# MIT-REALM/gcbf-pytorch

Hardware: NVIDIA H100
Metric: agent*steps/sec (train step, device-timed) (higher is better)
Workload: dtype f32 via 3xfp16 tensor-core products (fp32 accumulate)

## Files before the change

### gcbf-pytorch_b200/csrc/gemm_wgmma_f16.cu

```cuda
#include <cuda.h>
#include <cuda_fp16.h>
#include <stdlib.h>

#include <atomic>

#include "common.cuh"
#include "sm90_ptx.cuh"

namespace gcbf {
namespace th {

using namespace ptx;

constexpr int BM = 128;
constexpr int BK = 32;
constexpr int SUB_N = 128;
constexpr int WG_K = 16;
constexpr int NUM_THREADS = 384;
constexpr int EPI_THREADS = 256;
constexpr int KCH_MAX = 256 / BK;
constexpr int MN_BOX = 64;
constexpr int A_BYTES = BM * BK * 2;
constexpr int B_BYTES = SUB_N * BK * 2;
constexpr int RING_BYTES = 128 * 1024;
template <int P> __host__ __device__ constexpr int stage_bytes() { return P == 3 ? 2 * A_BYTES + 2 * B_BYTES : A_BYTES + B_BYTES; }
template <int P> __host__ __device__ constexpr int stages() { return RING_BYTES / stage_bytes<P>(); }
constexpr int PARK_PITCH = SUB_N + 8;
constexpr int PARK_BYTES = BM * PARK_PITCH * 4;
static_assert(PARK_BYTES <= RING_BYTES, "the second half of a 256-wide tile is parked in the stage ring");
static_assert(2 * stages<1>() * 8 + (256 / 32) * 4 <= 256, "barriers and reduction words fit their 256 bytes");
constexpr int SMEM_BYTES = RING_BYTES + PARK_BYTES + 1024  + 256 ;

enum { EPI_FWD = 0, EPI_DGRAD = 1, EPI_WGRAD = 2 };

struct EpiParams {
  int mode;
  const float* alpha;
  const float* bias;
  int act;
  const float* relu_src;
  int ld_relu;
  const __half* relu_hi;
  int ld_relu_h;
  int accumulate;
  size_t split_stride;
  const uint32_t* amax_a; int a_sr, a_sc;
  const uint32_t* amax_b; int b_sr, b_sc;
  uint32_t* amax_out;
  __half* out_h;
  int ld_out_h;
  uint32_t* out_tile_amax;
  int out_amax_stride;
  float* colsum;
};

__host__ __device__ __forceinline__ uint32_t scale_bits_from_amax(uint32_t amax_bits) {
  const int e = (int)((amax_bits >> 23) & 0xffu);
  if (e == 0 || e == 255) return 0x3f800000u;
  int se = 127 + 14 - (e - 127);
  se = se < 2 ? 2 : (se > 252 ? 252 : se);
  return (uint32_t)se << 23;
}
__host__ __device__ __forceinline__ uint32_t inv_pow2_bits(uint32_t s_bits) { return (uint32_t)(254 - (int)(s_bits >> 23)) << 23; }

template <bool MN_MAJOR>
__device__ __forceinline__ uint64_t tile_desc(uint32_t tile_addr, int kk) {
  if (MN_MAJOR) {
    return make_smem_desc(tile_addr + (uint32_t)(kk * WG_K * 128), BK * 128, 1024, 128);
  }
  return make_smem_desc(tile_addr + (uint32_t)(kk * WG_K * 2), 16, 8 * BK * 2, BK * 2);
}

template <bool MN_MAJOR>
__device__ __forceinline__ void load_tile(uint8_t* dst, const CUtensorMap* map, uint64_t* bar, int mn0, int k0, int rows) {
  if (MN_MAJOR) {
    for (int j = 0; j < rows / MN_BOX; ++j) tma_load_2d(dst + j * (BK * 128), map, bar, mn0 + j * MN_BOX, k0);
  } else {
    tma_load_2d(dst, map, bar, k0, mn0);
  }
}

__device__ __forceinline__ void epi_sync() { asm volatile("bar.sync 1, %0;" ::"n"(EPI_THREADS) : "memory"); }

template <int BN, bool A_MN, bool B_MN, int P>
__global__ void __launch_bounds__(NUM_THREADS, 1)
gemm_h_kernel(const __grid_constant__ CUtensorMap map_a_hi, const __grid_constant__ CUtensorMap map_a_lo,
              const __grid_constant__ CUtensorMap map_b_hi, const __grid_constant__ CUtensorMap map_b_lo,
              float* __restrict__ C, int ldc, int Mo, int No, int tiles_n, int kblocks_per_split, int kblocks_total, int KCH, EpiParams ep) {
  static_assert(P == 3 || P == 1, "products per k-slice: 3 (3xFP16) or 1 (fp16)");
  constexpr int STAGES = stages<P>();
  constexpr int STAGE_BYTES = stage_bytes<P>();
  constexpr int B_OFF = (P == 3 ? 2 : 1) * A_BYTES;
  constexpr int NSUB = BN / SUB_N;
  constexpr int MODE = A_MN ? EPI_WGRAD : (B_MN ? EPI_DGRAD : EPI_FWD);
  extern __shared__ uint8_t smem_raw[];
  uint8_t* smem = reinterpret_cast<uint8_t*>((reinterpret_cast<uintptr_t>(smem_raw) + 1023) & ~uintptr_t(1023));
  float* park0 = reinterpret_cast<float*>(smem + RING_BYTES);
  float* park1 = reinterpret_cast<float*>(smem);
  uint64_t* bars = reinterpret_cast<uint64_t*>(smem + RING_BYTES + PARK_BYTES);
  uint64_t* full = bars;
  uint64_t* empty = bars + STAGES;
  uint32_t* red = reinterpret_cast<uint32_t*>(bars + 2 * STAGES);

  const int warp = threadIdx.x >> 5, lane = threadIdx.x & 31;
  const int kb0 = blockIdx.y * kblocks_per_split;
  const int kb1 = min(kblocks_total, kb0 + kblocks_per_split);
  const int nkb = kb1 - kb0;
  const int m0 = (blockIdx.x / tiles_n) * BM, n0t = (blockIdx.x % tiles_n) * BN;

  if (threadIdx.x == 0) {
    tma_prefetch_desc(&map_a_hi);
    if (P == 3) tma_prefetch_desc(&map_a_lo);
    tma_prefetch_desc(&map_b_hi);
    if (P == 3) tma_prefetch_desc(&map_b_lo);
    for (int s = 0; s < STAGES; ++s) { mbar_init(&full[s], 1); mbar_init(&empty[s], 2); }
    fence_barrier_init();
  }
  __syncthreads();

  if (warp < 4) {
    setmaxnreg_dec<40>();
    if (threadIdx.x == 0) {
      int stage = 0;
      uint32_t phase = 0;
      for (int sub = 0; sub < NSUB; ++sub) {
        for (int kb = kb0; kb < kb1; ++kb) {
          mbar_wait(&empty[stage], phase ^ 1);
          uint8_t* st = smem + stage * STAGE_BYTES;
          mbar_expect_tx(&full[stage], STAGE_BYTES);
          load_tile<A_MN>(st, &map_a_hi, &full[stage], m0, kb * BK, BM);
          if (P == 3) load_tile<A_MN>(st + A_BYTES, &map_a_lo, &full[stage], m0, kb * BK, BM);
          load_tile<B_MN>(st + B_OFF, &map_b_hi, &full[stage], n0t + sub * SUB_N, kb * BK, SUB_N);
          if (P == 3) load_tile<B_MN>(st + B_OFF + B_BYTES, &map_b_lo, &full[stage], n0t + sub * SUB_N, kb * BK, SUB_N);
          if (++stage == STAGES) { stage = 0; phase ^= 1; }
        }
      }
    }
  } else {
    setmaxnreg_inc<232>();
    if (nkb > 0) {
      const int tid = threadIdx.x - 128;
      const int wg = tid >> 7;
      const int wl = (tid >> 5) & 3;
      const bool leader = (tid & 127) == 0;
      const uint32_t a_off = (uint32_t)wg * 4096u;
      const int nch = (nkb + KCH - 1) / KCH;
      int nchunks = NSUB * nch;
      asm("" : "+r"(nchunks));
      int stage = 0;
      uint32_t phase = 0;
      int held = -1;
      float cs_prev = 0.f;
      float acc[64], d0[64], d1[64];
#pragma unroll
      for (int j = 0; j < 64; ++j) acc[j] = 0.f;

      auto park_acc = [&](float* park) {
        const int r0 = wg * 64 + wl * 16 + (lane >> 2);
#pragma unroll
        for (int j = 0; j < 64; j += 4) {
          const int c = 8 * (j >> 2) + 2 * (lane & 3);
          *reinterpret_cast<float2*>(park + r0 * PARK_PITCH + c) = make_float2(acc[j], acc[j + 1]);
          *reinterpret_cast<float2*>(park + (r0 + 8) * PARK_PITCH + c) = make_float2(acc[j + 2], acc[j + 3]);
        }
      };
      auto promote = [&](float (&p)[64], float cs) {
#pragma unroll
        for (int j = 0; j < 64; ++j) fence_operand(p[j]);
#pragma unroll
        for (int j = 0; j < 64; ++j) acc[j] = __fmaf_rn(p[j], cs, acc[j]);
      };
      auto run_chunk = [&](float (&d)[64], float (&p)[64], int g) {
        const int sub = (NSUB > 1 && g >= nch) ? 1 : 0;
        const int kc = (g - sub * nch) * KCH;
        const int n0 = n0t + sub * SUB_N;
        const int kstart = (kb0 + kc) * BK;
        const int ia = A_MN ? (kstart >> 7) * ep.a_sr + (m0 >> 8) * ep.a_sc : (m0 >> 7) * ep.a_sr + (kstart >> 8) * ep.a_sc;
        const int ib = B_MN ? (kstart >> 7) * ep.b_sr + (n0 >> 8) * ep.b_sc : 0;
        const float cs = __uint_as_float(inv_pow2_bits(scale_bits_from_amax(__ldg(ep.amax_a + ia)))) *
                         __uint_as_float(inv_pow2_bits(scale_bits_from_amax(__ldg(ep.amax_b + ib))));
        const int kend = min(nkb, kc + KCH);
        for (int kb = kc; kb < kend; ++kb) {
          mbar_wait(&full[stage], phase);
          const uint32_t st = smem_u32(smem + stage * STAGE_BYTES);
          const uint32_t a_hi = st + a_off, a_lo = st + A_BYTES + a_off, b_hi = st + B_OFF, b_lo = st + B_OFF + B_BYTES;
#pragma unroll
          for (int j = 0; j < 64; ++j) fence_operand(d[j]);
          wgmma_fence();
#pragma unroll
          for (int kk = 0; kk < BK / WG_K; ++kk) {
            if constexpr (P == 3) {
              const uint64_t dah = tile_desc<A_MN>(a_hi, kk), dal = tile_desc<A_MN>(a_lo, kk);
              const uint64_t dbh = tile_desc<B_MN>(b_hi, kk), dbl = tile_desc<B_MN>(b_lo, kk);
              wgmma_m64n128k16_f16<A_MN ? 1 : 0, B_MN ? 1 : 0>(d, dal, dbh, (kb > kc || kk > 0) ? 1u : 0u);
              wgmma_m64n128k16_f16<A_MN ? 1 : 0, B_MN ? 1 : 0>(d, dah, dbl, 1u);
              wgmma_m64n128k16_f16<A_MN ? 1 : 0, B_MN ? 1 : 0>(d, dah, dbh, 1u);
            } else {
              const uint64_t dah = tile_desc<A_MN>(a_hi, kk), dbh = tile_desc<B_MN>(b_hi, kk);
              wgmma_m64n128k16_f16<A_MN ? 1 : 0, B_MN ? 1 : 0>(d, dah, dbh, (kb > kc || kk > 0) ? 1u : 0u);
            }
          }
          wgmma_commit();
          wgmma_wait<1>();
          if (held >= 0 && leader) mbar_arrive(&empty[held]);
          held = stage;
          if (++stage == STAGES) { stage = 0; phase ^= 1; }
          if (kb == kc && g > 0) {
            promote(p, cs_prev);
            if (NSUB > 1 && g == nch) {
              park_acc(park0);
#pragma unroll
              for (int j = 0; j < 64; ++j) acc[j] = 0.f;
            }
          }
        }
        cs_prev = cs;
      };
      auto finish = [&](float (&d)[64]) {
        wgmma_wait<0>();
        if (leader) mbar_arrive(&empty[held]);
        promote(d, cs_prev);
        if (NSUB > 1) epi_sync();
        park_acc(NSUB > 1 ? park1 : park0);
      };
      for (int g = 0;; g += 2) {
        run_chunk(d0, d1, g);
        if (g + 1 == nchunks) { finish(d0); break; }
        run_chunk(d1, d0, g + 1);
        if (g + 2 == nchunks) { finish(d1); break; }
      }
      epi_sync();

      constexpr int CG4 = BN / 4;
      constexpr int ROWS_PER_ITER = EPI_THREADS / CG4;
      const int cg = tid % CG4;
      const int c = cg * 4;
      const int col = n0t + c;
      float* const pk = (c < SUB_N ? park0 : park1) + (c & (SUB_N - 1));
      const float alpha = ep.alpha ? __ldg(ep.alpha) : 1.f;
      float bias4[4] = {0.f, 0.f, 0.f, 0.f};
      if (MODE == EPI_FWD && ep.bias) {
        const float inv_alpha = 1.f / alpha;
#pragma unroll
        for (int u = 0; u < 4; ++u) bias4[u] = (col + u < No) ? __ldg(ep.bias + col + u) * inv_alpha : 0.f;
      }
      float tmax = 0.f;
      for (int r = tid / CG4; r < BM; r += ROWS_PER_ITER) {
        const int row = m0 + r;
        float4* p = reinterpret_cast<float4*>(pk + r * PARK_PITCH);
        float v[4];
        const float4 s = *p;
        v[0] = s.x; v[1] = s.y; v[2] = s.z; v[3] = s.w;
#pragma unroll
        for (int u = 0; u < 4; ++u) {
          float y = (v[u] + bias4[u]) * alpha;
          if (MODE == EPI_FWD) {
            if (ep.act == GCBF_ACT_RELU) y = fmaxf(y, 0.f);
            else if (ep.act == GCBF_ACT_TANH) y = tanhf(y);
          }
          const bool ok = row < Mo && col + u < No;
          if (MODE == EPI_DGRAD && ok) {
            if (ep.relu_src) y = (__ldg(ep.relu_src + (size_t)row * ep.ld_relu + col + u) > 0.f) ? y : 0.f;
            else if (ep.relu_hi) y = (__half2float(ep.relu_hi[(size_t)row * ep.ld_relu_h + col + u]) > 0.f) ? y : 0.f;
          }
          v[u] = ok ? y : 0.f;
          tmax = fmaxf(tmax, fabsf(v[u]));
        }
        *p = make_float4(v[0], v[1], v[2], v[3]);
      }
      float s_tile = 1.f;
      if (MODE != EPI_WGRAD && ep.out_h) {
        const uint32_t wmax = __reduce_max_sync(0xffffffffu, __float_as_uint(tmax));
        if (lane == 0) red[tid >> 5] = wmax;
        epi_sync();
        uint32_t m = 0;
#pragma unroll
        for (int w = 0; w < EPI_THREADS / 32; ++w) m = max(m, red[w]);
        s_tile = __uint_as_float(scale_bits_from_amax(m));
        if (tid == 0 && m0 < Mo && n0t < No) ep.out_tile_amax[(size_t)(m0 >> 7) * ep.out_amax_stride + (n0t >> 8)] = m;
      }
      float out_max = 0.f;
      const bool vec_c = C && (ldc & 3) == 0 && (reinterpret_cast<uintptr_t>(C) & 15) == 0;
      const size_t plane = (size_t)Mo * ep.ld_out_h;
      for (int r = tid / CG4; r < BM; r += ROWS_PER_ITER) {
        const int row = m0 + r;
        if (row >= Mo || col >= No) continue;
        const float4 s = *reinterpret_cast<const float4*>(pk + r * PARK_PITCH);
        const float v[4] = {s.x, s.y, s.z, s.w};
        const int nv = min(4, No - col);
        if (C) {
          float* dst = C + (size_t)blockIdx.y * ep.split_stride + (size_t)row * ldc + col;
          if (ep.accumulate) {
#pragma unroll
            for (int u = 0; u < 4; ++u)
              if (u < nv) { const float o = v[u] + dst[u]; dst[u] = o; out_max = fmaxf(out_max, fabsf(o)); }
          } else if (vec_c && nv == 4) {
            *reinterpret_cast<float4*>(dst) = s;
          } else {
#pragma unroll
            for (int u = 0; u < 4; ++u)
              if (u < nv) dst[u] = v[u];
          }
        }
        if (MODE != EPI_WGRAD && ep.out_h) {
          const float y0 = v[0] * s_tile, y1 = v[1] * s_tile, y2 = v[2] * s_tile, y3 = v[3] * s_tile;
          const __half2 h01 = __floats2half2_rn(y0, y1), h23 = __floats2half2_rn(y2, y3);
          const float2 f01 = __half22float2(h01), f23 = __half22float2(h23);
          const __half2 l01 = __floats2half2_rn(__fsub_rn(y0, f01.x), __fsub_rn(y1, f01.y));
          const __half2 l23 = __floats2half2_rn(__fsub_rn(y2, f23.x), __fsub_rn(y3, f23.y));
          __half* dh = ep.out_h + (size_t)row * ep.ld_out_h + col;
          if (nv == 4) {
            *reinterpret_cast<uint2*>(dh) = make_uint2(*reinterpret_cast<const uint32_t*>(&h01), *reinterpret_cast<const uint32_t*>(&h23));
            *reinterpret_cast<uint2*>(dh + plane) = make_uint2(*reinterpret_cast<const uint32_t*>(&l01), *reinterpret_cast<const uint32_t*>(&l23));
          } else {
            const __half hs[4] = {__low2half(h01), __high2half(h01), __low2half(h23), __high2half(h23)};
            const __half ls[4] = {__low2half(l01), __high2half(l01), __low2half(l23), __high2half(l23)};
            for (int u = 0; u < nv; ++u) { dh[u] = hs[u]; dh[plane + u] = ls[u]; }
          }
        }
      }
      if (ep.amax_out && !ep.accumulate) out_max = fmaxf(out_max, tmax);
      if (MODE == EPI_DGRAD && ep.colsum) epi_sync();
      if (MODE == EPI_DGRAD && ep.colsum && tid < BN) {
        const float* pc = (tid < SUB_N ? park0 : park1) + (tid & (SUB_N - 1));
        float csum = 0.f;
#pragma unroll 8
        for (int r = 0; r < BM; ++r) csum += pc[r * PARK_PITCH];
        if (n0t + tid < No) ep.colsum[(size_t)(blockIdx.x / tiles_n) * No + n0t + tid] = csum;
      }
      if (ep.amax_out) {
        const uint32_t m = __reduce_max_sync(0xffffffffu, __float_as_uint(out_max));
        if (lane == 0 && m) atomicMax(ep.amax_out, m);
      }
    }
  }
}
__global__ void amax_kernel(const float* __restrict__ src, int ld, int rows, int cols, uint32_t* __restrict__ slot, int vec4) {
  float m = 0.f;
  if (vec4) {
    const int w = cols >> 2;
    for (int r = blockIdx.x; r < rows; r += gridDim.x) {
      const float4* p = reinterpret_cast<const float4*>(src + (size_t)r * ld);
      for (int c = threadIdx.x; c < w; c += blockDim.x) {
        const float4 x = __ldg(p + c);
        m = fmaxf(fmaxf(m, fmaxf(fabsf(x.x), fabsf(x.y))), fmaxf(fabsf(x.z), fabsf(x.w)));
      }
    }
  } else {
    for (int r = blockIdx.x; r < rows; r += gridDim.x)
      for (int c = threadIdx.x; c < cols; c += blockDim.x) m = fmaxf(m, fabsf(__ldg(src + (size_t)r * ld + c)));
  }
  const uint32_t w = __reduce_max_sync(0xffffffffu, __float_as_uint(m));
  __shared__ uint32_t part[32];
  if ((threadIdx.x & 31) == 0) part[threadIdx.x >> 5] = w;
  __syncthreads();
  if (threadIdx.x < 32) {
    uint32_t v = threadIdx.x < (blockDim.x >> 5) ? part[threadIdx.x] : 0u;
    v = __reduce_max_sync(0xffffffffu, v);
    if (threadIdx.x == 0 && v) atomicMax(slot, v);
  }
}

constexpr int SPLIT_ROWS = 64;
__global__ void split_h_kernel(const float* __restrict__ src, int ld, int rows, int cols, const uint32_t* __restrict__ amax,
                               __half* __restrict__ dst, int ld_h, float* __restrict__ colsum) {
  const float s = __uint_as_float(scale_bits_from_amax(__ldg(amax)));
  const int c = (blockIdx.x * 32 + threadIdx.x) * 2;
  const int r0 = blockIdx.y * SPLIT_ROWS;
  const size_t plane = (size_t)rows * ld_h;
  float s0 = 0.f, s1 = 0.f;
  if (c < cols) {
    const bool pair = (c + 1 < cols);
    const int r1 = min(rows, r0 + SPLIT_ROWS);
    for (int r = r0 + threadIdx.y; r < r1; r += blockDim.y) {
      const float* p = src + (size_t)r * ld + c;
      const float x0 = __ldg(p), x1 = pair ? __ldg(p + 1) : 0.f;
      const float y0 = x0 * s, y1 = x1 * s;
      const __half2 hi = __floats2half2_rn(y0, y1);
      const float2 hf = __half22float2(hi);
      const __half2 lo = __floats2half2_rn(__fsub_rn(y0, hf.x), __fsub_rn(y1, hf.y));
      __half* d = dst + (size_t)r * ld_h + c;
      if (pair) {
        *reinterpret_cast<__half2*>(d) = hi;
        *reinterpret_cast<__half2*>(d + plane) = lo;
      } else {
        d[0] = __low2half(hi);
        d[plane] = __low2half(lo);
      }
      s0 += x0; s1 += x1;
    }
  }
  if (colsum) {
    __shared__ float red[8][64];
    red[threadIdx.y][2 * threadIdx.x] = s0;
    red[threadIdx.y][2 * threadIdx.x + 1] = s1;
    __syncthreads();
    if (threadIdx.y == 0) {
      float t0 = 0.f, t1 = 0.f;
#pragma unroll
      for (int y = 0; y < 8; ++y) { t0 += red[y][2 * threadIdx.x]; t1 += red[y][2 * threadIdx.x + 1]; }
      if (c < cols) colsum[(size_t)blockIdx.y * cols + c] = t0;
      if (c + 1 < cols) colsum[(size_t)blockIdx.y * cols + c + 1] = t1;
    }
  }
}

__device__ __forceinline__ void split4(const float4 x, float s, uint2& hi, uint2& lo) {
  const float y0 = x.x * s, y1 = x.y * s, y2 = x.z * s, y3 = x.w * s;
  const __half2 h01 = __floats2half2_rn(y0, y1), h23 = __floats2half2_rn(y2, y3);
  const float2 f01 = __half22float2(h01), f23 = __half22float2(h23);
  const __half2 l01 = __floats2half2_rn(__fsub_rn(y0, f01.x), __fsub_rn(y1, f01.y));
  const __half2 l23 = __floats2half2_rn(__fsub_rn(y2, f23.x), __fsub_rn(y3, f23.y));
  hi.x = *reinterpret_cast<const uint32_t*>(&h01); hi.y = *reinterpret_cast<const uint32_t*>(&h23);
  lo.x = *reinterpret_cast<const uint32_t*>(&l01); lo.y = *reinterpret_cast<const uint32_t*>(&l23);
}

__global__ void __launch_bounds__(256) split_h4_kernel(const float* __restrict__ src, int ld, int rows, int cols,
                                                       const uint32_t* __restrict__ amax, __half* __restrict__ dst, int ld_h,
                                                       float* __restrict__ colsum) {
  const float s = __uint_as_float(scale_bits_from_amax(__ldg(amax)));
  const int c = (blockIdx.x * 32 + threadIdx.x) * 4;
  const int r0 = blockIdx.y * SPLIT_ROWS;
  const size_t plane = (size_t)rows * ld_h;
  float cs[4] = {0.f, 0.f, 0.f, 0.f};
  if (c < cols) {
    const int r1 = min(rows, r0 + SPLIT_ROWS);
    for (int r = r0 + threadIdx.y; r < r1; r += 32) {
      float4 x[4];
#pragma unroll
      for (int u = 0; u < 4; ++u)
        x[u] = (r + 8 * u < r1) ? __ldg(reinterpret_cast<const float4*>(src + (size_t)(r + 8 * u) * ld + c)) : make_float4(0.f, 0.f, 0.f, 0.f);
#pragma unroll
      for (int u = 0; u < 4; ++u) {
        if (r + 8 * u < r1) {
          uint2 hi, lo;
          split4(x[u], s, hi, lo);
          __half* d = dst + (size_t)(r + 8 * u) * ld_h + c;
          *reinterpret_cast<uint2*>(d) = hi;
          *reinterpret_cast<uint2*>(d + plane) = lo;
          cs[0] += x[u].x; cs[1] += x[u].y; cs[2] += x[u].z; cs[3] += x[u].w;
        }
      }
    }
  }
  if (colsum) {
    __shared__ float red[8][128];
#pragma unroll
    for (int j = 0; j < 4; ++j) red[threadIdx.y][4 * threadIdx.x + j] = cs[j];
    __syncthreads();
    if (threadIdx.y < 4) {
      const int col = threadIdx.y * 32 + threadIdx.x;
      float t = 0.f;
#pragma unroll
      for (int y = 0; y < 8; ++y) t += red[y][col];
      const int gc = blockIdx.x * 128 + col;
      if (gc < cols) colsum[(size_t)blockIdx.y * cols + gc] = t;
    }
  }
}

constexpr int kSplitMaxBatch = 16;
struct SplitBatch {
  const float* src[kSplitMaxBatch];
  uint32_t* amax[kSplitMaxBatch];
  __half* dst[kSplitMaxBatch];
  int ld[kSplitMaxBatch], rows[kSplitMaxBatch], cols[kSplitMaxBatch], ld_h[kSplitMaxBatch];
};

__global__ void __launch_bounds__(256) amax_batched_kernel(const __grid_constant__ SplitBatch b) {
  const int t = blockIdx.z;
  const int ld = b.ld[t], rows = b.rows[t], cols = b.cols[t];
  const int warp = threadIdx.x >> 5, lane = threadIdx.x & 31;
  const float* __restrict__ src = b.src[t];
  const bool vec = ((cols & 3) == 0 && (ld & 3) == 0 && (reinterpret_cast<uintptr_t>(src) & 15) == 0);
  float m = 0.f;
  for (int r = blockIdx.x * 8 + warp; r < rows; r += gridDim.x * 8) {
    const float* row = src + (size_t)r * ld;
    if (vec) {
      const float4* p = reinterpret_cast<const float4*>(row);
      for (int c = lane; c < (cols >> 2); c += 32) {
        const float4 x = __ldg(p + c);
        m = fmaxf(fmaxf(m, fmaxf(fabsf(x.x), fabsf(x.y))), fmaxf(fabsf(x.z), fabsf(x.w)));
      }
    } else {
      for (int c = lane; c < cols; c += 32) m = fmaxf(m, fabsf(__ldg(row + c)));
    }
  }
  const uint32_t w = __reduce_max_sync(0xffffffffu, __float_as_uint(m));
  __shared__ uint32_t part[8];
  if (lane == 0) part[warp] = w;
  __syncthreads();
  if (threadIdx.x < 32) {
    uint32_t v = threadIdx.x < 8 ? part[threadIdx.x] : 0u;
    v = __reduce_max_sync(0xffffffffu, v);
    if (threadIdx.x == 0 && v) atomicMax(b.amax[t], v);
  }
}

__global__ void __launch_bounds__(256) split_batched_kernel(const __grid_constant__ SplitBatch b) {
  const int t = blockIdx.z;
  const int ld = b.ld[t], rows = b.rows[t], cols = b.cols[t], ld_h = b.ld_h[t];
  const int c = (blockIdx.x * 32 + threadIdx.x) * 2;
  const int r0 = blockIdx.y * SPLIT_ROWS;
  if (c >= cols || r0 >= rows) return;
  const float* __restrict__ src = b.src[t];
  __half* __restrict__ dst = b.dst[t];
  const float s = __uint_as_float(scale_bits_from_amax(*b.amax[t]));
  const size_t plane = (size_t)rows * ld_h;
  const bool pair = (c + 1 < cols);
  const int r1 = min(rows, r0 + SPLIT_ROWS);
  for (int r = r0 + threadIdx.y; r < r1; r += blockDim.y) {
    const float* p = src + (size_t)r * ld + c;
    const float y0 = __ldg(p) * s, y1 = pair ? __ldg(p + 1) * s : 0.f;
    const __half2 hi = __floats2half2_rn(y0, y1);
    const float2 hf = __half22float2(hi);
    const __half2 lo = __floats2half2_rn(__fsub_rn(y0, hf.x), __fsub_rn(y1, hf.y));
    __half* d = dst + (size_t)r * ld_h + c;
    if (pair) {
      *reinterpret_cast<__half2*>(d) = hi;
      *reinterpret_cast<__half2*>(d + plane) = lo;
    } else {
      d[0] = __low2half(hi);
      d[plane] = __low2half(lo);
    }
  }
}

typedef CUresult (*EncodeTiledFn)(CUtensorMap*, CUtensorMapDataType, cuuint32_t, void*, const cuuint64_t*, const cuuint64_t*,
                                  const cuuint32_t*, const cuuint32_t*, CUtensorMapInterleave, CUtensorMapSwizzle,
                                  CUtensorMapL2promotion, CUtensorMapFloatOOBfill);

static EncodeTiledFn get_encode_fn() {
  static EncodeTiledFn fn = nullptr;
  if (!fn) {
    void* p = nullptr;
    cudaDriverEntryPointQueryResult q;
    if (cudaGetDriverEntryPoint("cuTensorMapEncodeTiled", &p, cudaEnableDefault, &q) == cudaSuccess && p) fn = (EncodeTiledFn)p;
  }
  return fn;
}

static int make_map(CUtensorMap* map, const __half* base, int rows, int cols, int ld_h, bool mn_major, int tile_rows) {
  EncodeTiledFn fn = get_encode_fn();
  if (!fn) { set_error("cuTensorMapEncodeTiled entry point unavailable"); return GCBF_E_CUDA; }
  cuuint64_t dims[2] = {(cuuint64_t)cols, (cuuint64_t)rows};
  cuuint64_t strides[1] = {(cuuint64_t)ld_h * 2};
  cuuint32_t box[2] = {(cuuint32_t)(mn_major ? MN_BOX : BK), (cuuint32_t)(mn_major ? BK : tile_rows)};
  cuuint32_t estr[2] = {1, 1};
  CUresult r = fn(map, CU_TENSOR_MAP_DATA_TYPE_FLOAT16, 2, const_cast<__half*>(base), dims, strides, box, estr,
                  CU_TENSOR_MAP_INTERLEAVE_NONE, mn_major ? CU_TENSOR_MAP_SWIZZLE_128B : CU_TENSOR_MAP_SWIZZLE_64B,
                  CU_TENSOR_MAP_L2_PROMOTION_L2_256B, CU_TENSOR_MAP_FLOAT_OOB_FILL_NONE);
  if (r != CUDA_SUCCESS) {
    set_error("cuTensorMapEncodeTiled failed (%d) rows=%d cols=%d ld=%d mn=%d", (int)r, rows, cols, ld_h, (int)mn_major);
    return GCBF_E_CUDA;
  }
  return GCBF_OK;
}

static std::atomic<long long> g_tc_launches[2];

static bool g_env_read = false;
static int g_kch = 4;
static int g_kch_dgrad = 8;

struct Operand {
  const __half* hi; int rows; int cols; int ld_h; bool mn_major;
  const __half* lo() const { return hi + (size_t)rows * ld_h; }
};
struct OutH {
  __half* hi; int rows; int cols; int ld_h; uint32_t* tile_amax; int amax_stride;
};

template <int BN, bool A_MN, bool B_MN, int P>
static int launch(const Operand& A, const Operand& B, float* C, int ldc, int Mo, int No, int Kc, int splits, EpiParams ep,
                  const OutH* oh, cudaStream_t st) {
  if (!g_env_read) {
    const char* kc = getenv("GCBF_TC_KCH");
    if (kc && atoi(kc) >= 1 && atoi(kc) <= KCH_MAX) g_kch = atoi(kc);
    const char* kd = getenv("GCBF_TC_KCH_DGRAD");
    if (kd && atoi(kd) >= 1 && atoi(kd) <= KCH_MAX) g_kch_dgrad = atoi(kd);
    if (kc && !kd) g_kch_dgrad = g_kch > 4 ? g_kch : g_kch_dgrad;
    g_env_read = true;
  }
  if ((ep.a_sr || ep.a_sc || ep.b_sr || ep.b_sc) && g_kch > 4) { set_error("tile-scaled operands need promotion chunks of <= 128 K-elements (GCBF_TC_KCH <= 4)"); return GCBF_E_UNSUPPORTED; }
  if constexpr (BN != 256 || A_MN) {
    if (oh || ep.colsum) { set_error("companion emission / column sums need a 256-wide forward or data-grad launch"); return GCBF_E_UNSUPPORTED; }
  }
  CUtensorMap mah, mal, mbh, mbl;
  if (int rc = make_map(&mah, A.hi, A.rows, A.cols, A.ld_h, A_MN, BM)) return rc;
  if (int rc = make_map(&mbh, B.hi, B.rows, B.cols, B.ld_h, B_MN, SUB_N)) return rc;
  if (P == 3) {
    if (int rc = make_map(&mal, A.lo(), A.rows, A.cols, A.ld_h, A_MN, BM)) return rc;
    if (int rc = make_map(&mbl, B.lo(), B.rows, B.cols, B.ld_h, B_MN, SUB_N)) return rc;
  } else {
    mal = mah; mbl = mbh;
  }
  if (oh) {
    ep.out_h = oh->hi; ep.ld_out_h = oh->ld_h; ep.out_tile_amax = oh->tile_amax; ep.out_amax_stride = oh->amax_stride;
  }
  static bool attr_set = false;
  if (!attr_set) {
    GCBF_CUDA_OK(cudaFuncSetAttribute(gemm_h_kernel<BN, A_MN, B_MN, P>, cudaFuncAttributeMaxDynamicSharedMemorySize, SMEM_BYTES));
    attr_set = true;
  }
  const int tiles_m = ceil_div(Mo, BM), tiles_n = ceil_div(No, BN);
  const int kblocks = ceil_div(Kc, BK);
  const int kch = (!A_MN && B_MN && !(ep.b_sr || ep.b_sc)) ? g_kch_dgrad : g_kch;
  const int kps = ceil_div(ceil_div(kblocks, splits), kch) * kch;
  const int nsplit = ceil_div(kblocks, kps);
  float* part = nullptr;
  float* colsum_part = nullptr;
  float* const colsum = ep.colsum;
  const int accumulate = ep.accumulate;
  if (nsplit > 1) {
    GCBF_CUDA_OK(scratch_alloc((void**)&part, (size_t)nsplit * Mo * No * 4, st));
    ep.split_stride = (size_t)Mo * No;
    ep.accumulate = 0;
  }
  if (colsum) {
    GCBF_CUDA_OK(scratch_alloc((void**)&colsum_part, (size_t)tiles_m * No * 4, st));
    ep.colsum = colsum_part;
  }
  gemm_h_kernel<BN, A_MN, B_MN, P><<<dim3(tiles_m * tiles_n, nsplit), NUM_THREADS, SMEM_BYTES, st>>>(mah, mal, mbh, mbl, part ? part : C,
                                                                                                    part ? No : ldc, Mo, No, tiles_n, kps,
                                                                                                    kblocks, kch, ep);
  GCBF_LAUNCH_OK();
  g_tc_launches[P == 1 ? 1 : 0].fetch_add(1, std::memory_order_relaxed);
  if (part) {
    GCBF_CUDA_OK(add_partials(part, nsplit, Mo, No, C, ldc, accumulate, st));
    GCBF_CUDA_OK(scratch_free(part, st));
  }
  if (colsum_part) {
    GCBF_CUDA_OK(add_partials(colsum_part, tiles_m, 1, No, colsum, No, 1, st));
    GCBF_CUDA_OK(scratch_free(colsum_part, st));
  }
  return GCBF_OK;
}

template <int BN, bool A_MN, bool B_MN>
static int launch_p(int products, const Operand& A, const Operand& B, float* C, int ldc, int Mo, int No, int Kc, int splits,
                    const EpiParams& ep, const OutH* oh, cudaStream_t st) {
  return products == 1 ? launch<BN, A_MN, B_MN, 1>(A, B, C, ldc, Mo, No, Kc, splits, ep, oh, st)
                       : launch<BN, A_MN, B_MN, 3>(A, B, C, ldc, Mo, No, Kc, splits, ep, oh, st);
}

static int check_plane(const void* p, int ld_h, const char* what) {
  if (!p || (reinterpret_cast<uintptr_t>(p) & 15) || (ld_h & 7)) {
    set_error("%s: fp16 companion must be 16-byte aligned with a pitch that is a multiple of 8 halves (ptr=%p ld=%d)", what, p, ld_h);
    return GCBF_E_INVALID;
  }
  return GCBF_OK;
}

}
}

using namespace gcbf;

extern "C" int gcbf_amax_f32(const float* src, int ld, int rows, int cols, void* amax_slot, int accumulate, void* stream) {
  GCBF_REQUIRE(amax_slot && rows >= 0 && cols >= 0 && ld >= cols, "gcbf_amax_f32: bad arguments rows=%d cols=%d ld=%d", rows, cols, ld);
  cudaStream_t st = as_stream(stream);
  if (!accumulate) GCBF_CUDA_OK(cudaMemsetAsync(amax_slot, 0, 4, st));
  if (rows == 0 || cols == 0) return GCBF_OK;
  GCBF_REQUIRE(src, "gcbf_amax_f32: null src");
  const int vec4 = ((cols & 3) == 0 && (ld & 3) == 0 && (reinterpret_cast<uintptr_t>(src) & 15) == 0) ? 1 : 0;
  const int work = vec4 ? cols / 4 : cols;
  const int threads = work >= 256 ? 256 : (work >= 128 ? 128 : 64);
  const int blocks = (int)imin64(rows, (int64_t)kNumSMs * (2048 / threads));
  th::amax_kernel<<<blocks, threads, 0, st>>>(src, ld, rows, cols, reinterpret_cast<uint32_t*>(amax_slot), vec4);
  GCBF_LAUNCH_OK();
  return GCBF_OK;
}

extern "C" int gcbf_split_f16(const float* src, int ld, int rows, int cols, const void* amax_slot, void* dst, int ld_h,
                              float* colsum, int colsum_accumulate, void* stream) {
  GCBF_REQUIRE(amax_slot && dst && rows >= 0 && cols >= 0 && ld >= cols && ld_h >= cols, "gcbf_split_f16: bad arguments rows=%d cols=%d", rows, cols);
  if (int rc = th::check_plane(dst, ld_h, "gcbf_split_f16")) return rc;
  cudaStream_t st = as_stream(stream);
  if (colsum && !colsum_accumulate) GCBF_CUDA_OK(cudaMemsetAsync(colsum, 0, (size_t)cols * 4, st));
  if (rows == 0 || cols == 0) return GCBF_OK;
  GCBF_REQUIRE(src, "gcbf_split_f16: null src");
  dim3 block(32, 8);
  const int strips = ceil_div(rows, th::SPLIT_ROWS);
  float* part = nullptr;
  if (colsum) GCBF_CUDA_OK(scratch_alloc((void**)&part, (size_t)strips * cols * 4, st));
  if ((cols & 3) == 0 && (ld & 3) == 0 && (reinterpret_cast<uintptr_t>(src) & 15) == 0) {
    dim3 grid(ceil_div(cols, 128), strips);
    th::split_h4_kernel<<<grid, block, 0, st>>>(src, ld, rows, cols, reinterpret_cast<const uint32_t*>(amax_slot),
                                               reinterpret_cast<__half*>(dst), ld_h, part);
  } else {
    dim3 grid(ceil_div(cols, 64), strips);
    th::split_h_kernel<<<grid, block, 0, st>>>(src, ld, rows, cols, reinterpret_cast<const uint32_t*>(amax_slot),
                                              reinterpret_cast<__half*>(dst), ld_h, part);
  }
  GCBF_LAUNCH_OK();
  if (part) {
    GCBF_CUDA_OK(add_partials(part, strips, 1, cols, colsum, cols, 1, st));
    GCBF_CUDA_OK(scratch_free(part, st));
  }
  return GCBF_OK;
}

extern "C" int gcbf_amax_split_batched(const gcbf_split_desc* descs, int count, void* stream) {
  GCBF_REQUIRE(descs && count >= 0, "gcbf_amax_split_batched: bad arguments");
  cudaStream_t st = as_stream(stream);
  for (int base = 0; base < count; base += th::kSplitMaxBatch) {
    const int nb = min(th::kSplitMaxBatch, count - base);
    th::SplitBatch b{};
    int max_rows = 0, max_cols = 0;
    for (int i = 0; i < nb; ++i) {
      const gcbf_split_desc& d = descs[base + i];
      GCBF_REQUIRE(d.src && d.amax_slot && d.dst && d.rows > 0 && d.cols > 0 && d.ld >= d.cols && d.ld_h >= d.cols,
                   "gcbf_amax_split_batched: descriptor %d", base + i);
      if (int rc = th::check_plane(d.dst, d.ld_h, "gcbf_amax_split_batched")) return rc;
      b.src[i] = d.src; b.amax[i] = reinterpret_cast<uint32_t*>(d.amax_slot); b.dst[i] = reinterpret_cast<__half*>(d.dst);
      b.ld[i] = d.ld; b.rows[i] = d.rows; b.cols[i] = d.cols; b.ld_h[i] = d.ld_h;
      max_rows = max(max_rows, d.rows); max_cols = max(max_cols, d.cols);
      GCBF_CUDA_OK(cudaMemsetAsync(d.amax_slot, 0, 4, st));
    }
    th::amax_batched_kernel<<<dim3(min(ceil_div(max_rows, 8), 8 * kNumSMs), 1, nb), 256, 0, st>>>(b);
    GCBF_LAUNCH_OK();
    th::split_batched_kernel<<<dim3(ceil_div(max_cols, 64), ceil_div(max_rows, th::SPLIT_ROWS), nb), dim3(32, 8), 0, st>>>(b);
    GCBF_LAUNCH_OK();
  }
  return GCBF_OK;
}

extern "C" long long gcbf_tc_launch_count(int products, int reset) {
  if (products != 1 && products != 3) { set_error("gcbf_tc_launch_count: products %d (3 or 1)", products); return -1; }
  std::atomic<long long>& c = th::g_tc_launches[products == 1 ? 1 : 0];
  return reset ? c.exchange(0) : c.load();
}

extern "C" int gcbf_linear_h_supported(int M, int N, int K) {
  return (M >= 256 && N >= 96 && K >= 96 && (long long)M * N * K >= (1ll << 24)) ? 1 : 0;
}

static int check_h16(const gcbf_h16* h, const char* what, int rows, int cols) {
  if (!h || !h->buf || !h->amax || h->rows != rows || h->cols != cols || h->ld < cols) {
    set_error("%s: companion descriptor (expected [%d x %d])", what, rows, cols);
    return GCBF_E_INVALID;
  }
  return th::check_plane(h->buf, h->ld, what);
}

extern "C" int gcbf_linear_fwd_tp(const gcbf_h16* X, const gcbf_h16* W, const float* bias, const float* inv_sigma, int act, float* Y, int ldy,
                                  const gcbf_h16* Yh, void* out_amax, int M, int N, int K, void* stream, int products) {
  GCBF_REQUIRE(M > 0 && N > 0 && K > 0 && (Y || Yh) && (!Y || ldy >= N), "gcbf_linear_fwd_t: bad arguments M=%d N=%d K=%d", M, N, K);
  GCBF_REQUIRE(products == 3 || products == 1, "gcbf_linear_fwd_tp: products %d (3 or 1)", products);
  if (int rc = check_h16(X, "gcbf_linear_fwd_t X", M, K)) return rc;
  if (int rc = check_h16(W, "gcbf_linear_fwd_t W", N, K)) return rc;
  GCBF_REQUIRE(W->amax_row_stride == 0 && W->amax_col_stride == 0, "gcbf_linear_fwd_t: the weight companion must be per-tensor scaled");
  cudaStream_t st = as_stream(stream);
  th::EpiParams ep{};
  ep.mode = th::EPI_FWD; ep.alpha = inv_sigma; ep.bias = bias; ep.act = act;
  ep.amax_a = reinterpret_cast<const uint32_t*>(X->amax); ep.a_sr = X->amax_row_stride; ep.a_sc = X->amax_col_stride;
  ep.amax_b = reinterpret_cast<const uint32_t*>(W->amax);
  ep.amax_out = reinterpret_cast<uint32_t*>(out_amax);
  if (out_amax) GCBF_CUDA_OK(cudaMemsetAsync(out_amax, 0, 4, st));
  th::OutH oh{};
  if (Yh) {
    if (int rc = check_h16(Yh, "gcbf_linear_fwd_t Yh", M, N)) return rc;
    GCBF_REQUIRE(N > 128 && Yh->amax_row_stride == ceil_div(N, 256) && Yh->amax_col_stride == 1, "gcbf_linear_fwd_t: emitted companions are tile-scaled (N > 128, amax strides (ceil(N/256), 1))");
    oh = th::OutH{reinterpret_cast<__half*>(Yh->buf), M, N, Yh->ld, reinterpret_cast<uint32_t*>(Yh->amax), Yh->amax_row_stride};
  }
  th::Operand A{reinterpret_cast<const __half*>(X->buf), M, K, X->ld, false}, B{reinterpret_cast<const __half*>(W->buf), N, K, W->ld, false};
  return (N > 128) ? th::launch_p<256, false, false>(products, A, B, Y, ldy, M, N, K, 1, ep, Yh ? &oh : nullptr, st)
                   : th::launch_p<128, false, false>(products, A, B, Y, ldy, M, N, K, 1, ep, nullptr, st);
}

extern "C" int gcbf_linear_fwd_t(const gcbf_h16* X, const gcbf_h16* W, const float* bias, const float* inv_sigma, int act, float* Y, int ldy,
                                 const gcbf_h16* Yh, void* out_amax, int M, int N, int K, void* stream) {
  return gcbf_linear_fwd_tp(X, W, bias, inv_sigma, act, Y, ldy, Yh, out_amax, M, N, K, stream, 3);
}

extern "C" int gcbf_linear_bwd_data_tp(const gcbf_h16* dZ, const gcbf_h16* W, const float* inv_sigma, const float* relu_src, int ld_relu,
                                       const gcbf_h16* relu_h, float* dX, int lddx, int accumulate, const gcbf_h16* dXh, float* colsum,
                                       void* out_amax, int M, int N, int K, void* stream, int products) {
  GCBF_REQUIRE(M > 0 && N > 0 && K > 0 && (dX || dXh) && (!dX || lddx >= K), "gcbf_linear_bwd_data_t: bad arguments M=%d N=%d K=%d", M, N, K);
  GCBF_REQUIRE(products == 3 || products == 1, "gcbf_linear_bwd_data_tp: products %d (3 or 1)", products);
  GCBF_REQUIRE(!relu_src || ld_relu >= K, "gcbf_linear_bwd_data_t: ld_relu");
  GCBF_REQUIRE(!(relu_src && relu_h) && !(accumulate && (dXh || colsum)), "gcbf_linear_bwd_data_t: conflicting options");
  if (int rc = check_h16(dZ, "gcbf_linear_bwd_data_t dZ", M, N)) return rc;
  if (int rc = check_h16(W, "gcbf_linear_bwd_data_t W", N, K)) return rc;
  GCBF_REQUIRE(W->amax_row_stride == 0 && W->amax_col_stride == 0, "gcbf_linear_bwd_data_t: the weight companion must be per-tensor scaled");
  if (relu_h) { if (int rc = check_h16(relu_h, "gcbf_linear_bwd_data_t relu_h", M, K)) return rc; }
  cudaStream_t st = as_stream(stream);
  th::EpiParams ep{};
  ep.mode = th::EPI_DGRAD; ep.alpha = inv_sigma; ep.relu_src = relu_src; ep.ld_relu = ld_relu; ep.accumulate = accumulate;
  if (relu_h) { ep.relu_hi = reinterpret_cast<const __half*>(relu_h->buf); ep.ld_relu_h = relu_h->ld; }
  ep.amax_a = reinterpret_cast<const uint32_t*>(dZ->amax); ep.a_sr = dZ->amax_row_stride; ep.a_sc = dZ->amax_col_stride;
  ep.amax_b = reinterpret_cast<const uint32_t*>(W->amax);
  ep.amax_out = reinterpret_cast<uint32_t*>(out_amax);
  ep.colsum = colsum;
  if (out_amax) GCBF_CUDA_OK(cudaMemsetAsync(out_amax, 0, 4, st));
  th::OutH oh{};
  if (dXh) {
    if (int rc = check_h16(dXh, "gcbf_linear_bwd_data_t dXh", M, K)) return rc;
    GCBF_REQUIRE(K > 128 && dXh->amax_row_stride == ceil_div(K, 256) && dXh->amax_col_stride == 1, "gcbf_linear_bwd_data_t: emitted companions are tile-scaled (K > 128, amax strides (ceil(K/256), 1))");
    oh = th::OutH{reinterpret_cast<__half*>(dXh->buf), M, K, dXh->ld, reinterpret_cast<uint32_t*>(dXh->amax), dXh->amax_row_stride};
  }
  th::Operand A{reinterpret_cast<const __half*>(dZ->buf), M, N, dZ->ld, false}, B{reinterpret_cast<const __half*>(W->buf), N, K, W->ld, true};
  return (K > 128) ? th::launch_p<256, false, true>(products, A, B, dX, lddx, M, K, N, 1, ep, dXh ? &oh : nullptr, st)
                   : th::launch_p<128, false, true>(products, A, B, dX, lddx, M, K, N, 1, ep, nullptr, st);
}

extern "C" int gcbf_linear_bwd_data_t(const gcbf_h16* dZ, const gcbf_h16* W, const float* inv_sigma, const float* relu_src, int ld_relu,
                                      const gcbf_h16* relu_h, float* dX, int lddx, int accumulate, const gcbf_h16* dXh, float* colsum,
                                      void* out_amax, int M, int N, int K, void* stream) {
  return gcbf_linear_bwd_data_tp(dZ, W, inv_sigma, relu_src, ld_relu, relu_h, dX, lddx, accumulate, dXh, colsum, out_amax, M, N, K, stream, 3);
}

extern "C" int gcbf_linear_bwd_weight_tp(const gcbf_h16* dZ, const gcbf_h16* X, const float* inv_sigma, float* dW, int lddw, int accumulate,
                                         int M, int N, int K, void* stream, int products) {
  GCBF_REQUIRE(M > 0 && N > 0 && K > 0 && lddw >= K && dW, "gcbf_linear_bwd_weight_t: bad arguments M=%d N=%d K=%d", M, N, K);
  GCBF_REQUIRE(products == 3 || products == 1, "gcbf_linear_bwd_weight_tp: products %d (3 or 1)", products);
  if (int rc = check_h16(dZ, "gcbf_linear_bwd_weight_t dZ", M, N)) return rc;
  if (int rc = check_h16(X, "gcbf_linear_bwd_weight_t X", M, K)) return rc;
  cudaStream_t st = as_stream(stream);
  th::EpiParams ep{};
  ep.mode = th::EPI_WGRAD; ep.alpha = inv_sigma; ep.accumulate = accumulate;
  ep.amax_a = reinterpret_cast<const uint32_t*>(dZ->amax); ep.a_sr = dZ->amax_row_stride; ep.a_sc = dZ->amax_col_stride;
  ep.amax_b = reinterpret_cast<const uint32_t*>(X->amax); ep.b_sr = X->amax_row_stride; ep.b_sc = X->amax_col_stride;
  const int BN = (K > 128) ? 256 : 128;
  const int tiles = ceil_div(N, th::BM) * ceil_div(K, BN);
  int splits = 1;
  if (tiles < kNumSMs) splits = max(1, min(ceil_div(M, 256), kNumSMs / tiles));
  th::Operand A{reinterpret_cast<const __half*>(dZ->buf), M, N, dZ->ld, true}, B{reinterpret_cast<const __half*>(X->buf), M, K, X->ld, true};
  return (BN == 256) ? th::launch_p<256, true, true>(products, A, B, dW, lddw, N, K, M, splits, ep, nullptr, st)
                     : th::launch_p<128, true, true>(products, A, B, dW, lddw, N, K, M, splits, ep, nullptr, st);
}

extern "C" int gcbf_linear_bwd_weight_t(const gcbf_h16* dZ, const gcbf_h16* X, const float* inv_sigma, float* dW, int lddw, int accumulate,
                                        int M, int N, int K, void* stream) {
  return gcbf_linear_bwd_weight_tp(dZ, X, inv_sigma, dW, lddw, accumulate, M, N, K, stream, 3);
}

static gcbf_h16 per_tensor(const void* buf, int ld, const void* amax, int rows, int cols) {
  gcbf_h16 h;
  h.buf = const_cast<void*>(buf); h.amax = const_cast<void*>(amax); h.ld = ld; h.rows = rows; h.cols = cols; h.amax_row_stride = 0; h.amax_col_stride = 0;
  return h;
}

extern "C" int gcbf_linear_fwd_h(const void* Xh, int ldxh, const void* x_amax, const void* Wh, int ldwh, const void* w_amax,
                                 const float* bias, const float* inv_sigma, float* Y, int ldy, int M, int N, int K, int act,
                                 void* out_amax, void* stream) {
  GCBF_REQUIRE(Y && x_amax && w_amax, "gcbf_linear_fwd_h: null pointer");
  const gcbf_h16 X = per_tensor(Xh, ldxh, x_amax, M, K), W = per_tensor(Wh, ldwh, w_amax, N, K);
  return gcbf_linear_fwd_t(&X, &W, bias, inv_sigma, act, Y, ldy, nullptr, out_amax, M, N, K, stream);
}

extern "C" int gcbf_linear_bwd_data_h(const void* dZh, int lddzh, const void* dz_amax, const void* Wh, int ldwh,
                                      const void* w_amax, const float* inv_sigma, const float* relu_src, int ld_relu, float* dX,
                                      int lddx, int M, int N, int K, int accumulate, void* out_amax, void* stream) {
  GCBF_REQUIRE(dX && dz_amax && w_amax, "gcbf_linear_bwd_data_h: null pointer");
  const gcbf_h16 dZ = per_tensor(dZh, lddzh, dz_amax, M, N), W = per_tensor(Wh, ldwh, w_amax, N, K);
  return gcbf_linear_bwd_data_t(&dZ, &W, inv_sigma, relu_src, ld_relu, nullptr, dX, lddx, accumulate, nullptr, nullptr, out_amax, M, N, K, stream);
}

extern "C" int gcbf_linear_bwd_weight_h(const void* dZh, int lddzh, const void* dz_amax, const void* Xh, int ldxh,
                                        const void* x_amax, const float* inv_sigma, float* dW, int lddw, int M, int N, int K,
                                        int accumulate, void* stream) {
  GCBF_REQUIRE(dW && dz_amax && x_amax, "gcbf_linear_bwd_weight_h: null pointer");
  const gcbf_h16 dZ = per_tensor(dZh, lddzh, dz_amax, M, N), X = per_tensor(Xh, ldxh, x_amax, M, K);
  return gcbf_linear_bwd_weight_t(&dZ, &X, inv_sigma, dW, lddw, accumulate, M, N, K, stream);
}
```

### gcbf-pytorch_b200/csrc/sm90_ptx.cuh

```cuda
#pragma once
#include <cuda.h>
#include <stdint.h>

namespace gcbf {
namespace ptx {

__device__ __forceinline__ uint32_t smem_u32(const void* p) { return (uint32_t)__cvta_generic_to_shared(p); }

__device__ __forceinline__ void mbar_init(uint64_t* bar, uint32_t count) {
  asm volatile("mbarrier.init.shared::cta.b64 [%0], %1;" ::"r"(smem_u32(bar)), "r"(count));
}
__device__ __forceinline__ void mbar_expect_tx(uint64_t* bar, uint32_t bytes) {
  asm volatile("mbarrier.arrive.expect_tx.shared::cta.b64 _, [%0], %1;" ::"r"(smem_u32(bar)), "r"(bytes) : "memory");
}
__device__ __forceinline__ void mbar_arrive(uint64_t* bar) {
  asm volatile("mbarrier.arrive.shared::cta.b64 _, [%0];" ::"r"(smem_u32(bar)) : "memory");
}
__device__ __forceinline__ uint32_t mbar_try_wait(uint64_t* bar, uint32_t parity) {
  uint32_t ok;
  asm volatile(
      "{\n\t"
      ".reg .pred p;\n\t"
      "mbarrier.try_wait.parity.shared::cta.b64 p, [%1], %2;\n\t"
      "selp.u32 %0, 1, 0, p;\n\t"
      "}"
      : "=r"(ok)
      : "r"(smem_u32(bar)), "r"(parity)
      : "memory");
  return ok;
}
__device__ __forceinline__ void mbar_wait(uint64_t* bar, uint32_t parity) {
  while (!mbar_try_wait(bar, parity)) {
  }
}
__device__ __forceinline__ void fence_barrier_init() { asm volatile("fence.mbarrier_init.release.cluster;" ::: "memory"); }

__device__ __forceinline__ void tma_load_2d(void* smem_dst, const CUtensorMap* map, uint64_t* bar, int c0, int c1) {
  asm volatile(
      "cp.async.bulk.tensor.2d.shared::cluster.global.mbarrier::complete_tx::bytes [%0], [%1, {%3, %4}], [%2];" ::"r"(
          smem_u32(smem_dst)),
      "l"(reinterpret_cast<uint64_t>(map)), "r"(smem_u32(bar)), "r"(c0), "r"(c1)
      : "memory");
}
__device__ __forceinline__ void tma_prefetch_desc(const CUtensorMap* map) {
  asm volatile("prefetch.tensormap [%0];" ::"l"(reinterpret_cast<uint64_t>(map)) : "memory");
}

__device__ __forceinline__ void wgmma_fence() { asm volatile("wgmma.fence.sync.aligned;" ::: "memory"); }
__device__ __forceinline__ void wgmma_commit() { asm volatile("wgmma.commit_group.sync.aligned;" ::: "memory"); }
template <int N>
__device__ __forceinline__ void wgmma_wait() { asm volatile("wgmma.wait_group.sync.aligned %0;" ::"n"(N) : "memory"); }
__device__ __forceinline__ void fence_operand(float& r) { asm volatile("" : "+f"(r)::"memory"); }

template <int R>
__device__ __forceinline__ void setmaxnreg_dec() { asm volatile("setmaxnreg.dec.sync.aligned.u32 %0;" ::"n"(R)); }
template <int R>
__device__ __forceinline__ void setmaxnreg_inc() { asm volatile("setmaxnreg.inc.sync.aligned.u32 %0;" ::"n"(R)); }

template <int TA, int TB>
__device__ __forceinline__ void wgmma_m64n128k16_f16(float (&d)[64], uint64_t desc_a, uint64_t desc_b, uint32_t scale_d) {
  asm volatile(
      "{\n\t"
      ".reg .pred p;\n\t"
      "setp.ne.b32 p, %66, 0;\n\t"
      "wgmma.mma_async.sync.aligned.m64n128k16.f32.f16.f16 "
      "{%0, %1, %2, %3, %4, %5, %6, %7, %8, %9, %10, %11, %12, %13, %14, %15, "
      "%16, %17, %18, %19, %20, %21, %22, %23, %24, %25, %26, %27, %28, %29, %30, %31, "
      "%32, %33, %34, %35, %36, %37, %38, %39, %40, %41, %42, %43, %44, %45, %46, %47, "
      "%48, %49, %50, %51, %52, %53, %54, %55, %56, %57, %58, %59, %60, %61, %62, %63}, "
      "%64, %65, p, 1, 1, %67, %68;\n\t"
      "}\n"
      : "+f"(d[0]), "+f"(d[1]), "+f"(d[2]), "+f"(d[3]), "+f"(d[4]), "+f"(d[5]), "+f"(d[6]), "+f"(d[7]), "+f"(d[8]), "+f"(d[9]),
        "+f"(d[10]), "+f"(d[11]), "+f"(d[12]), "+f"(d[13]), "+f"(d[14]), "+f"(d[15]), "+f"(d[16]), "+f"(d[17]), "+f"(d[18]),
        "+f"(d[19]), "+f"(d[20]), "+f"(d[21]), "+f"(d[22]), "+f"(d[23]), "+f"(d[24]), "+f"(d[25]), "+f"(d[26]), "+f"(d[27]),
        "+f"(d[28]), "+f"(d[29]), "+f"(d[30]), "+f"(d[31]), "+f"(d[32]), "+f"(d[33]), "+f"(d[34]), "+f"(d[35]), "+f"(d[36]),
        "+f"(d[37]), "+f"(d[38]), "+f"(d[39]), "+f"(d[40]), "+f"(d[41]), "+f"(d[42]), "+f"(d[43]), "+f"(d[44]), "+f"(d[45]),
        "+f"(d[46]), "+f"(d[47]), "+f"(d[48]), "+f"(d[49]), "+f"(d[50]), "+f"(d[51]), "+f"(d[52]), "+f"(d[53]), "+f"(d[54]),
        "+f"(d[55]), "+f"(d[56]), "+f"(d[57]), "+f"(d[58]), "+f"(d[59]), "+f"(d[60]), "+f"(d[61]), "+f"(d[62]), "+f"(d[63])
      : "l"(desc_a), "l"(desc_b), "r"(scale_d), "n"(TA), "n"(TB)
      : "memory");
}

__device__ __forceinline__ uint64_t make_smem_desc(uint32_t smem_addr, uint32_t lbo_bytes, uint32_t sbo_bytes, int swizzle_bytes) {
  uint64_t d = 0;
  d |= (uint64_t)((smem_addr >> 4) & 0x3FFF);
  d |= (uint64_t)((lbo_bytes >> 4) & 0x3FFF) << 16;
  d |= (uint64_t)((sbo_bytes >> 4) & 0x3FFF) << 32;
  d |= (uint64_t)(swizzle_bytes == 128 ? 1 : swizzle_bytes == 64 ? 2 : swizzle_bytes == 32 ? 3 : 0) << 62;
  return d;
}

}
}
```

Baseline: 363,100.

## Prefetch ReLU mask into L2 and batch-load it into bitmask in dgrad epilogue

The producer thread issues bulk L2 prefetches for the ReLU mask rows of the output tile early in the mainloop. The epilogue then loads the mask with vectorized loads for all rows up front and packs it into per-thread bitmasks, replacing scattered scalar loads inside the per-element loop. It also drops an epilogue barrier in the colsum path when a half-precision output is written, presumably because an earlier sync already covers it. The cost is extra registers and more producer-thread work, plus the risk that the dropped sync was still needed.

New measurement: 386,000, median of 6. 6.3% higher.

```diff
diff --git a/gcbf-pytorch_b200/csrc/gemm_wgmma_f16.cu b/gcbf-pytorch_b200/csrc/gemm_wgmma_f16.cu
--- a/gcbf-pytorch_b200/csrc/gemm_wgmma_f16.cu
+++ b/gcbf-pytorch_b200/csrc/gemm_wgmma_f16.cu
@@ -121,6 +121,16 @@
   if (warp < 4) {
     setmaxnreg_dec<40>();
     if (threadIdx.x == 0) {
+      bool mask_pending = MODE == EPI_DGRAD && (ep.relu_hi || ep.relu_src);
+      auto prefetch_mask = [&]() {
+        const int cols = min(BN, No - n0t), rows = min(BM, Mo - m0);
+        const bool vec = !ep.relu_src || ((ep.ld_relu & 3) == 0 && (reinterpret_cast<uintptr_t>(ep.relu_src) & 15) == 0);
+        const uint32_t bytes = (uint32_t)(cols * (ep.relu_src ? 4 : 2)) & ~15u;
+        if (vec && bytes)
+          for (int r = 0; r < rows; ++r)
+            bulk_prefetch_l2(ep.relu_src ? static_cast<const void*>(ep.relu_src + (size_t)(m0 + r) * ep.ld_relu + n0t)
+                                         : static_cast<const void*>(ep.relu_hi + (size_t)(m0 + r) * ep.ld_relu_h + n0t), bytes);
+      };
       int stage = 0;
       uint32_t phase = 0;
       for (int sub = 0; sub < NSUB; ++sub) {
@@ -133,6 +143,7 @@
           load_tile<B_MN>(st + B_OFF, &map_b_hi, &full[stage], n0t + sub * SUB_N, kb * BK, SUB_N);
           if (P == 3) load_tile<B_MN>(st + B_OFF + B_BYTES, &map_b_lo, &full[stage], n0t + sub * SUB_N, kb * BK, SUB_N);
           if (++stage == STAGES) { stage = 0; phase ^= 1; }
+          if (mask_pending && (stage == 0 || kb + 1 == kb1)) { prefetch_mask(); mask_pending = false; }
         }
       }
     }
@@ -244,8 +255,64 @@
 #pragma unroll
         for (int u = 0; u < 4; ++u) bias4[u] = (col + u < No) ? __ldg(ep.bias + col + u) * inv_alpha : 0.f;
       }
+      constexpr int RPT = BM / ROWS_PER_ITER;
+      const bool has_mask = MODE == EPI_DGRAD && (ep.relu_src || ep.relu_hi);
+      uint32_t mbits[RPT / 8];
+#pragma unroll
+      for (int w = 0; w < RPT / 8; ++w) mbits[w] = 0u;
+      if (has_mask && col < No) {
+        const int nv = min(4, No - col);
+        const bool vec = nv == 4 && (!ep.relu_src || ((ep.ld_relu & 3) == 0 && (reinterpret_cast<uintptr_t>(ep.relu_src) & 15) == 0));
+        uint4 raw[RPT];
+#pragma unroll
+        for (int i = 0; i < RPT; ++i) {
+          const int row = m0 + tid / CG4 + i * ROWS_PER_ITER;
+          raw[i] = make_uint4(0u, 0u, 0u, 0u);
+          if (row >= Mo) continue;
+          if (!ep.relu_src) {
+            const __half* q = ep.relu_hi + (size_t)row * ep.ld_relu_h + col;
+            if (vec) {
+              const uint2 h = __ldg(reinterpret_cast<const uint2*>(q));
+              raw[i].x = h.x; raw[i].y = h.y;
+            } else {
+              const unsigned short* qs = reinterpret_cast<const unsigned short*>(q);
+              raw[i].x = __ldg(qs);
+              if (nv > 1) raw[i].x |= (uint32_t)__ldg(qs + 1) << 16;
+              if (nv > 2) raw[i].y = __ldg(qs + 2);
+            }
+          } else {
+            const float* q = ep.relu_src + (size_t)row * ep.ld_relu + col;
+            if (vec) {
+              const float4 f = __ldg(reinterpret_cast<const float4*>(q));
+              raw[i] = make_uint4(__float_as_uint(f.x), __float_as_uint(f.y), __float_as_uint(f.z), __float_as_uint(f.w));
+            } else {
+              raw[i].x = __float_as_uint(__ldg(q));
+              if (nv > 1) raw[i].y = __float_as_uint(__ldg(q + 1));
+              if (nv > 2) raw[i].z = __float_as_uint(__ldg(q + 2));
+              if (nv > 3) raw[i].w = __float_as_uint(__ldg(q + 3));
+            }
+          }
+        }
+#pragma unroll
+        for (int i = 0; i < RPT; ++i) {
+          float x[4];
+          if (!ep.relu_src) {
+            const float2 a = __half22float2(*reinterpret_cast<const __half2*>(&raw[i].x));
+            const float2 b = __half22float2(*reinterpret_cast<const __half2*>(&raw[i].y));
+            x[0] = a.x; x[1] = a.y; x[2] = b.x; x[3] = b.y;
+          } else {
+            x[0] = __uint_as_float(raw[i].x); x[1] = __uint_as_float(raw[i].y);
+            x[2] = __uint_as_float(raw[i].z); x[3] = __uint_as_float(raw[i].w);
+          }
+#pragma unroll
+          for (int u = 0; u < 4; ++u)
+            if (x[u] > 0.f) mbits[i / 8] |= 1u << (4 * (i % 8) + u);
+        }
+      }
       float tmax = 0.f;
-      for (int r = tid / CG4; r < BM; r += ROWS_PER_ITER) {
+#pragma unroll
+      for (int i = 0; i < RPT; ++i) {
+        const int r = tid / CG4 + i * ROWS_PER_ITER;
         const int row = m0 + r;
         float4* p = reinterpret_cast<float4*>(pk + r * PARK_PITCH);
         float v[4];
@@ -259,10 +326,7 @@
             else if (ep.act == GCBF_ACT_TANH) y = tanhf(y);
           }
           const bool ok = row < Mo && col + u < No;
-          if (MODE == EPI_DGRAD && ok) {
-            if (ep.relu_src) y = (__ldg(ep.relu_src + (size_t)row * ep.ld_relu + col + u) > 0.f) ? y : 0.f;
-            else if (ep.relu_hi) y = (__half2float(ep.relu_hi[(size_t)row * ep.ld_relu_h + col + u]) > 0.f) ? y : 0.f;
-          }
+          if (has_mask && ok) y = ((mbits[i / 8] >> (4 * (i % 8) + u)) & 1u) ? y : 0.f;
           v[u] = ok ? y : 0.f;
           tmax = fmaxf(tmax, fabsf(v[u]));
         }
@@ -320,7 +384,7 @@
         }
       }
       if (ep.amax_out && !ep.accumulate) out_max = fmaxf(out_max, tmax);
-      if (MODE == EPI_DGRAD && ep.colsum) epi_sync();
+      if (MODE == EPI_DGRAD && ep.colsum && !ep.out_h) epi_sync();
       if (MODE == EPI_DGRAD && ep.colsum && tid < BN) {
         const float* pc = (tid < SUB_N ? park0 : park1) + (tid & (SUB_N - 1));
         float csum = 0.f;
diff --git a/gcbf-pytorch_b200/csrc/sm90_ptx.cuh b/gcbf-pytorch_b200/csrc/sm90_ptx.cuh
--- a/gcbf-pytorch_b200/csrc/sm90_ptx.cuh
+++ b/gcbf-pytorch_b200/csrc/sm90_ptx.cuh
@@ -44,6 +44,9 @@
 }
 __device__ __forceinline__ void tma_prefetch_desc(const CUtensorMap* map) {
   asm volatile("prefetch.tensormap [%0];" ::"l"(reinterpret_cast<uint64_t>(map)) : "memory");
+}
+__device__ __forceinline__ void bulk_prefetch_l2(const void* gptr, uint32_t bytes) {
+  asm volatile("cp.async.bulk.prefetch.L2.global [%0], %1;" ::"l"(reinterpret_cast<uint64_t>(gptr)), "r"(bytes) : "memory");
 }
 
 __device__ __forceinline__ void wgmma_fence() { asm volatile("wgmma.fence.sync.aligned;" ::: "memory"); }
```
